# jyakaranda/A-LeGO-LOAM

Hardware: AMD Instinct MI355X
Metric: scans/sec (16x1800 LiDAR) full IP->LO->LM loop (higher is better)
Workload: dtype f32/f64

## Files before the change

### a-lego-loam_amd/csrc/kernels_lm.hip

```cpp
#include "dev_cost.h"
#include "prof.h"
#include "kf_store.h"
#include "gmap.h"
#include "vgrid.h"

#define LM_BLOCK 256

DEV_INLINE double* ldp(const LmCtx& L, int slot) { return L.ld + (size_t)slot * LD_COUNT; }
DEV_INLINE int* lip(const LmCtx& L, int slot) { return L.li + (size_t)slot * LI_COUNT; }

DEV_INLINE void lm_map_update(const LmCtx& L, int slot, int* li, int merge) {
  const int nkf = li[LI_NKF];
  if (nkf == 0) return;
  int* rec = L.rec + (size_t)slot * L.K;
  const int cnt = li[LI_REC_CNT];
  bool changed = false;
  if (cnt < L.K) {
    const int nk = min(nkf, L.K);
    changed = li[LI_DIRTY] != 0;
    for (int j = 0; j < nk; ++j) rec[j] = nkf - nk + j;
    li[LI_REC_CNT] = nk;
  } else if (li[LI_LATEST] != nkf - 1) {
    for (int j = 0; j + 1 < L.K; ++j) rec[j] = rec[j + 1];
    rec[L.K - 1] = nkf - 1;
// ... 82 lines not shown
  if (j >= nk) return;
  const int* rec = L.rec + (size_t)slot * L.K;
  int offc = 0, offs = 0;
  for (int i = 0; i < j; ++i) { const int* kc = kf_cnt_of(L, kf_row(L, slot, rec[i])); offc += kc[KF_CORNER]; offs += kc[KF_SURF] + kc[KF_OUTL]; }
  const KfRingRow R = kf_ring_row_at(L, slot, kf_entry(L, rec[j]), KF_CORNER);
  const int nc = R.cnt[KF_CORNER], ns = R.cnt[KF_SURF], no = R.cnt[KF_OUTL];
  float m[3][4];
  keypose_matrix(R.pose, m);
  const float4 *sc_ = R.raw, *ss_ = kf_raw_of(L, R.row, KF_SURF), *so_ = kf_raw_of(L, R.row, KF_OUTL);
  float4* dc = L.map_corner_raw + (size_t)slot * L.map_cap_c + offc;
  float4* ds = L.map_surf_raw + (size_t)slot * L.map_cap_s + offs;
  for (int i = blockIdx.x * LM_BLOCK + threadIdx.x; i < nc; i += gridDim.x * LM_BLOCK) dc[i] = kf_transform(m, sc_[i]);
  for (int i = blockIdx.x * LM_BLOCK + threadIdx.x; i < ns; i += gridDim.x * LM_BLOCK) ds[i] = kf_transform(m, ss_[i]);
  for (int i = blockIdx.x * LM_BLOCK + threadIdx.x; i < no; i += gridDim.x * LM_BLOCK) ds[ns + i] = kf_transform(m, so_[i]);
  if (j == nk - 1 && blockIdx.x == 0 && threadIdx.x == 0) { li[LI_KRAW_C] = offc + nc; li[LI_KRAW_S] = offs + ns + no; }
}

__global__ void __launch_bounds__(LM_BLOCK) lm_total(DevCtx d, LmCtx L) {
  const int slot = blockIdx.y + d.slot0;
  int* li = lip(L, slot);
  if (!li[LI_RUN]) return;
  int ns = li[LI_NCUR_S], no = li[LI_NCUR_O];
  if (ns + no > L.total_cap) { no = L.total_cap - ns; if (threadIdx.x == 0 && blockIdx.x == 0) li[LI_OVERFLOW] = 1; }
  const float4* s = L.cur_surf_ds + (size_t)slot * L.kf_cap_s;
  const float4* o = L.cur_outl_ds + (size_t)slot * L.kf_cap_o;
  float4* t = L.cur_total + (size_t)slot * L.total_cap;
  for (int i = blockIdx.x * LM_BLOCK + threadIdx.x; i < ns; i += gridDim.x * LM_BLOCK) t[i] = s[i];
  for (int i = blockIdx.x * LM_BLOCK + threadIdx.x; i < no; i += gridDim.x * LM_BLOCK) t[ns + i] = o[i];
  if (blockIdx.x == 0 && threadIdx.x == 0) li[LI_NTOTAL] = ns + no;
}

DEV_INLINE int cell_coord(float x, float inv) { return (int)fminf(fmaxf(floorf(x * inv), -1073741824.0f), 1073741824.0f); }
DEV_INLINE int grid_cell(const GridGeom& g, float x, float y, float z, int* cx, int* cy, int* cz) {
  int ix = cell_coord(x, g.inv) - g.ox, iy = cell_coord(y, g.inv) - g.oy, iz = cell_coord(z, g.inv) - g.oz;
  *cx = ix; *cy = iy; *cz = iz;
  ix = min(max(ix, 0), g.gx - 1); iy = min(max(iy, 0), g.gy - 1); iz = min(max(iz, 0), g.gz - 1);
  return ix + g.gx * (iy + g.gy * iz);
}

__global__ void __launch_bounds__(LM_BLOCK) lm_grid_build(DevCtx d, LmCtx L) {
  const int slot = blockIdx.y + d.slot0, m = blockIdx.x;
  const int* li = lip(L, slot);
  if (!li[LI_REBUILD]) return;
  __shared__ GridGeom s_g;
// ... 782 lines not shown
  return hipFuncSetAttribute(reinterpret_cast<const void*>(lm_solve), hipFuncAttributeMaxDynamicSharedMemorySize, (int)LM_SOLVE_DYN_BYTES) == hipSuccess ? 0 : -1;
}

void launch_lm_prepare(const DevCtx& d, const LmCtx& L, int stage, int run_hint, int par, hipStream_t st) {
  const bool small = run_hint == 0 || stage == 2;
  const dim3 grid = small ? dim3(1, 1, d.n_launch) : dim3(8, 3, d.n_launch);
  ALEGO_LAUNCH(lm_prepare, grid, dim3(small ? 64 : LM_BLOCK), 0, st, d, L, stage, run_hint, par);
}
void launch_lm_stage(const DevCtx& d, const LmCtx& L, int run_hint, int par, hipStream_t st) {
  const dim3 grid = run_hint == 0 ? dim3(1, 1, d.n_launch) : dim3(8, 3, d.n_launch);
  ALEGO_LAUNCH(lm_stage, grid, dim3(run_hint == 0 ? 64 : LM_BLOCK), 0, st, d, L, run_hint, par);
}
void launch_lm_concat(const DevCtx& d, const LmCtx& L, hipStream_t st) {
  ALEGO_LAUNCH(lm_concat, dim3(2, L.K, d.n_launch), dim3(LM_BLOCK), 0, st, d, L);
}
void launch_lm_total(const DevCtx& d, const LmCtx& L, hipStream_t st) {
  ALEGO_LAUNCH(lm_total, dim3(8, d.n_launch), dim3(LM_BLOCK), 0, st, d, L);
}
void launch_lm_grid(const DevCtx& d, const LmCtx& L, hipStream_t st) {
  ALEGO_LAUNCH(lm_grid_build, dim3(2, d.n_launch), dim3(LM_BLOCK), 0, st, d, L);
}
int launch_lm_register(const DevCtx& d, const LmCtx& L, hipStream_t st, int (*allreduce)(void*, double*, size_t, hipStream_t), void* ar_ctx) {
  ALEGO_LAUNCH(lm_knn, dim3(lm_reg_grid(d, LM_ASSOC_GX)), dim3(128), 0, st, d, L);
  ALEGO_LAUNCH(lm_fit, dim3(lm_reg_grid(d, LM_FIT_GX)), dim3(128), 0, st, d, L);
  if (allreduce) {
    double* part = L.shard_part + (size_t)d.slot0 * 32;
    const size_t cnt = (size_t)d.n_launch * 32;
    const dim3 g1((d.n_launch + 63) / 64), b1(64);
    const int pre_next = d.P.lm_max_iters <= 0 ? (int)LM_PRE_STEP_FIRST_NEXT : (int)LM_PRE_STEP_NEXT;
    for (int outer = 0; outer < d.P.lm_outer_iters; ++outer) {
      ALEGO_LAUNCH(lm_shard_eval, dim3(d.n_launch), dim3(LM_SOLVE_T), LM_SOLVE_RED_BYTES, st, d, L, 0, outer == 0 ? (int)LM_PRE_PACK : pre_next);
      if (int rc = allreduce(ar_ctx, part, cnt, st)) return rc;
      for (int it = 0; it < d.P.lm_max_iters; ++it) {
// ... 21 lines not shown
```

### a-lego-loam_amd/csrc/kernels_voxel.hip

```cpp
#include <algorithm>
#include <cstring>

#include <hip/hip_runtime.h>

#include <vector>

#include "voxel.h"
#include "wave.h"
#include "vgrid.h"
#include "guard_alloc.h"
#include "prof.h"

typedef unsigned long long u64;

__device__ __forceinline__ bool vx_enabled(const VoxJob& J) { return J.enable == nullptr || *J.enable != 0; }

#ifndef VX_SMALL_MAX
#define VX_SMALL_MAX 8192
#endif

#ifndef VG_T
#define VG_T 512
#endif
#define VG_W (VG_T / 64)
#define VG_DMAX 9
#define VG_ND (1 << VG_DMAX)
#define VG_U 4

__device__ __forceinline__ int vg_div(int pos, int seglen, double inv_seglen) {
  int q = (int)((double)pos * inv_seglen);
  if (q * seglen > pos) --q;
  if ((q + 1) * seglen <= pos) ++q;
  return q;
}

#ifdef ALEGO_TIMING
__device__ long long vg_times[16];
#define VG_TICK(k) do { if (threadIdx.x == 0 && blockIdx.x == 0) vg_times[k] = wall_clock64(); } while (0)
#else
#define VG_TICK(k)
#endif
#define VG_LDS_BYTES ((2 * VG_W * VG_ND + VG_ND + 6 * VG_W + VG_W + 2 * (VG_W + 1)) * 4)
__device__ void vox_big_job(const VoxCtx& V, int job, unsigned char* smem) {
  const VoxJob J = V.jobs[job];
  const int n = min(*J.n_in, J.cap);
  const int tid = threadIdx.x, lane = tid & 63, wave = tid >> 6;
  typedef int cnt_t[VG_W][VG_ND];
  cnt_t* s_cnt = reinterpret_cast<cnt_t*>(smem);
  int* s_tot = reinterpret_cast<int*>(smem) + 2 * VG_W * VG_ND;
  typedef float red_t[VG_W];
  red_t* s_red = reinterpret_cast<red_t*>(s_tot + VG_ND);
  int* s_w = reinterpret_cast<int*>(s_red + 6);
  int* s_wbase = s_w + VG_W;
  int* s_nextfirst = s_wbase + VG_W + 1;
  const float inv = 1.0f / J.leaf;
  VG_TICK(0);
  float mn[3] = {3.402823466e+38f, 3.402823466e+38f, 3.402823466e+38f}, mx[3] = {-3.402823466e+38f, -3.402823466e+38f, -3.402823466e+38f};
  for (int i0 = tid; i0 < n; i0 += VG_T * VG_U) {
    float4 p[VG_U];
#pragma unroll
    for (int k = 0; k < VG_U; ++k) p[k] = J.in[min(i0 + k * VG_T, n - 1)];
#pragma unroll
    for (int k = 0; k < VG_U; ++k) vgr_box_add(mn, mx, p[k]);
  }
#pragma unroll
  for (int a = 0; a < 3; ++a) {
    bfly_minmax_f32(mn[a], mx[a]);
    if (lane == 0) { s_red[a][wave] = mn[a]; s_red[3 + a][wave] = mx[a]; }
  }
  __syncthreads();
#pragma unroll
  for (int a = 0; a < 3; ++a) {
    mn[a] = s_red[a][0]; mx[a] = s_red[3 + a][0];
#pragma unroll
    for (int w = 1; w < VG_W; ++w) { mn[a] = fminf(mn[a], s_red[a][w]); mx[a] = fmaxf(mx[a], s_red[3 + a][w]); }
  }
  if (tid < 3) {
    unsigned* bb = V.bbox + job * 8;
    bb[tid] = vgr_enc(tid == 0 ? mn[0] : tid == 1 ? mn[1] : mn[2]);
    bb[4 + tid] = ~vgr_enc(tid == 0 ? mx[0] : tid == 1 ? mx[1] : mx[2]);
  }
  const int sel = (J.mode == 1 && J.out_sel) ? *J.out_sel : 0;
  float4* const outp = J.out + (size_t)sel * (J.mode == 1 ? J.out_stride : 0);
  if (J.mode == 1 && tid < 6 && J.box_out) J.box_out[(size_t)sel * 8 + (tid < 3 ? tid : tid + 1)] = tid == 0 ? mn[0] : tid == 1 ? mn[1] : tid == 2 ? mn[2] : tid == 3 ? mx[0] : tid == 4 ? mx[1] : mx[2];
  if (vgr_leaf_too_small(mn, mx, inv)) {
    for (int i = tid; i < min(n, J.out_cap); i += VG_T) outp[i] = J.in[i];
    if (tid == 0) { *J.n_out = min(n, J.out_cap); if (n > J.out_cap && J.overflow) *J.overflow = 1;
                    if (J.mode == 1 && J.n_sel_out) J.n_sel_out[(size_t)sel * J.n_sel_stride] = min(n, J.out_cap); }
    return;
  }
  const VgrGeom g = vgr_geom(mn, mx, inv);
  const int bits = max(vgr_bits(g.T), 1);
  const int P = (bits + VG_DMAX - 1) / VG_DMAX, D = (bits + P - 1) / P, nd = 1 << D;
  const unsigned dmask = (unsigned)(nd - 1);
  const int seglen = ((n + VG_T - 1) / VG_T) * 64;
  const double inv_seglen = 1.0 / (double)seglen;
  const int seg0 = min(n, wave * seglen), seg1 = min(n, seg0 + seglen);
  unsigned* keys = V.keys + J.off;
  u64* bufA = V.pairs_a + J.off;
  u64* bufB = V.pairs_b + J.off;
  VG_TICK(1);
  for (int q = lane; q < VG_ND; q += 64) { s_cnt[0][wave][q] = 0; }
  for (int r0 = seg0 + lane; r0 < seg1; r0 += 64 * VG_U) {
    float4 pt[VG_U];
#pragma unroll
    for (int k = 0; k < VG_U; ++k) pt[k] = J.in[min(r0 + 64 * k, n - 1)];
#pragma unroll
    for (int k = 0; k < VG_U; ++k) {
      const int i = r0 + 64 * k;
      if (i < seg1) {
        const unsigned key = vgr_id(g, pt[k], inv);
        keys[i] = key;
        atomicAdd(&s_cnt[0][wave][key & dmask], 1);
      }
    }
  }
  VG_TICK(2);
  for (int p = 0; p < P; ++p) {
    const int cur = p & 1, nxt = cur ^ 1;
    const int sh = p * D, shn = (p + 1) * D;
    const u64* src = (p & 1) ? bufA : bufB;
// ... 46 lines not shown
        if (valid) {
          const int pos = my[dg] + s_tot[dg] + rank;
          dst[pos] = e[k];
          if (p + 1 < P) atomicAdd(&s_cnt[nxt][vg_div(pos, seglen, inv_seglen)][(key >> shn) & dmask], 1);
        }
        if (valid && rank == 0) my[dg] += (int)__popcll(m);
      }
    }
    VG_TICK(4 + 2 * p);
  }
  const u64* srt = (P & 1) ? bufA : bufB;
  __threadfence_block();
  __syncthreads();
  VG_TICK(11);
  if (J.mode == 1) {
    for (int i = tid; i < min(n, J.out_cap); i += VG_T) outp[i] = J.in[(unsigned)srt[i]];
    if (tid == 0) { *J.n_out = min(n, J.out_cap); if (n > J.out_cap && J.overflow) *J.overflow = 1;
                    if (J.n_sel_out) J.n_sel_out[(size_t)sel * J.n_sel_stride] = min(n, J.out_cap); }
    __syncthreads();
    return;
  }
  auto head_rounds = [&](int r0, bool* head) {
    u64 cur[VG_U], prv[VG_U];
#pragma unroll
    for (int k = 0; k < VG_U; ++k) {
      const int i = r0 + 64 * k + lane;
      cur[k] = srt[min(i, n - 1)]; prv[k] = srt[max(min(i, n - 1) - 1, 0)];
    }
#pragma unroll
    for (int k = 0; k < VG_U; ++k) {
      const int i = r0 + 64 * k + lane;
// ... 28 lines not shown
  VG_TICK(12);
  for (int r = tid; r < min(nvox, J.out_cap); r += VG_T) {
    int w = 0;
#pragma unroll
    for (int q = 1; q < VG_W; ++q) w += (r >= s_wbase[q]) ? 1 : 0;
    const int loc = r - s_wbase[w], ws0 = min(n, w * seglen);
    const int a = hl[ws0 + loc], bn = hl[ws0 + min(loc + 1, s_w[w] - 1)];
    const int b = loc + 1 < s_w[w] ? bn : s_nextfirst[w + 1];
    float sx = 0.f, sy = 0.f, sz = 0.f, si = 0.f;
    for (int j = a; j < b; j += 8) {
      unsigned q[8];
      float4 pt[8];
#pragma unroll
      for (int k = 0; k < 8; ++k) q[k] = (unsigned)srt[min(j + k, b - 1)];
#pragma unroll
      for (int k = 0; k < 8; ++k) pt[k] = J.in[q[k]];
#pragma unroll
      for (int k = 0; k < 8; ++k) if (j + k < b) { sx += pt[k].x; sy += pt[k].y; sz += pt[k].z; si += pt[k].w; }
    }
    const float fn = (float)(b - a);
    J.out[r] = make_float4(sx / fn, sy / fn, sz / fn, si / fn);
  }
  if (tid == 0) { *J.n_out = min(nvox, J.out_cap); if (nvox > J.out_cap && J.overflow) *J.overflow = 1; }
  __syncthreads();
  VG_TICK(13);
}
#ifdef ALEGO_TIMING
extern "C" void alego_vg_times(long long* out) { (void)hipMemcpyFromSymbol(out, HIP_SYMBOL(vg_times), sizeof(long long) * 16); }
#endif

#define VX_SB 512
#define VS_W (VX_SB / 64)
#define VS_DMAX 9
#define VS_ND (1 << VS_DMAX)
__device__ __forceinline__ bool vx_less(const unsigned* key, unsigned a, unsigned b) { return key[a] < key[b] || (key[a] == key[b] && a < b); }

__device__ void vox_small_job(const VoxCtx& V, int job) {
  const VoxJob J = V.jobs[job];
  const int n = min(*J.n_in, J.cap);
  const int tid = threadIdx.x, lane = tid & 63, wave = tid >> 6;
  extern __shared__ __attribute__((aligned(16))) unsigned char vs_smem[];
  unsigned* s_key = reinterpret_cast<unsigned*>(vs_smem);
  unsigned short* s_ia = reinterpret_cast<unsigned short*>(vs_smem + 4 * VX_SMALL_MAX);
  unsigned short* s_ib = reinterpret_cast<unsigned short*>(vs_smem + 6 * VX_SMALL_MAX);
  unsigned short* s_cnt = reinterpret_cast<unsigned short*>(vs_smem + 8 * VX_SMALL_MAX);
  __shared__ float s_red[6][VX_SB / 64];
  __shared__ int s_scan[VX_SB / 64];
  __shared__ int s_tot[VS_ND];
  const int sel = (J.mode == 1 && J.out_sel) ? *J.out_sel : 0;
  float4* const outp = J.out + (size_t)sel * (J.mode == 1 ? J.out_stride : 0);
  if (n == 0) { if (tid == 0) { *J.n_out = 0; if (J.mode == 1 && J.n_sel_out) J.n_sel_out[(size_t)sel * J.n_sel_stride] = 0; } return; }
  const float inv = 1.0f / J.leaf;
  VG_TICK(0);
  float mn[3] = {3.402823466e+38f, 3.402823466e+38f, 3.402823466e+38f}, mx[3] = {-3.402823466e+38f, -3.402823466e+38f, -3.402823466e+38f};
  for (int i = tid; i < n; i += VX_SB) vgr_box_add(mn, mx, J.in[i]);
#pragma unroll
  for (int a = 0; a < 3; ++a) {
    bfly_minmax_f32(mn[a], mx[a]);
    if (lane == 0) { s_red[a][wave] = mn[a]; s_red[3 + a][wave] = mx[a]; }
  }
  __syncthreads();
#pragma unroll
  for (int a = 0; a < 3; ++a) {
    mn[a] = s_red[a][0]; mx[a] = s_red[3 + a][0];
#pragma unroll
    for (int w = 1; w < VX_SB / 64; ++w) { mn[a] = fminf(mn[a], s_red[a][w]); mx[a] = fmaxf(mx[a], s_red[3 + a][w]); }
  }
  if (tid < 3) {
    unsigned* bb = V.bbox + job * 8;
    bb[tid] = vgr_enc(tid == 0 ? mn[0] : tid == 1 ? mn[1] : mn[2]);
    bb[4 + tid] = ~vgr_enc(tid == 0 ? mx[0] : tid == 1 ? mx[1] : mx[2]);
  }
  if (J.mode == 1 && tid < 6 && J.box_out) J.box_out[(size_t)sel * 8 + (tid < 3 ? tid : tid + 1)] = tid == 0 ? mn[0] : tid == 1 ? mn[1] : tid == 2 ? mn[2] : tid == 3 ? mx[0] : tid == 4 ? mx[1] : mx[2];
  if (vgr_leaf_too_small(mn, mx, inv)) {
    for (int i = tid; i < min(n, J.out_cap); i += VX_SB) outp[i] = J.in[i];
    if (tid == 0) { *J.n_out = min(n, J.out_cap); if (n > J.out_cap && J.overflow) *J.overflow = 1;
                    if (J.mode == 1 && J.n_sel_out) J.n_sel_out[(size_t)sel * J.n_sel_stride] = min(n, J.out_cap); }
    return;
  }
  VG_TICK(1);
  const VgrGeom g = vgr_geom(mn, mx, inv);
  for (int i = tid; i < n; i += VX_SB) s_key[i] = vgr_id(g, J.in[i], inv);
  VG_TICK(2);
  const int bits = max(vgr_bits(g.T), 1);
  const int P = (bits + VS_DMAX - 1) / VS_DMAX, D = (bits + P - 1) / P, nd = 1 << D;
  const unsigned dmask = (unsigned)(nd - 1);
  const int seglen = ((n + VX_SB - 1) / VX_SB) * 64;
  const int seg0 = min(n, wave * seglen), seg1 = min(n, seg0 + seglen);
  unsigned short* my = s_cnt + wave * VS_ND;
  for (int p = 0; p < P; ++p) {
    const unsigned short* src = (p & 1) ? s_ia : s_ib;
    unsigned short* dst = (p & 1) ? s_ib : s_ia;
    const int sh = p * D;
    __syncthreads();
    for (int q = lane; q < nd; q += 64) my[q] = 0;
    for (int sweep = 0; sweep < 2; ++sweep) {
      if (sweep == 1) {
        __syncthreads();
        if (tid < nd) {
          int run = 0;
#pragma unroll
          for (int w = 0; w < VS_W; ++w) { const int c = s_cnt[w * VS_ND + tid]; s_cnt[w * VS_ND + tid] = (unsigned short)run; run += c; }
          s_tot[tid] = run;
        }
        __syncthreads();
        if (wave == 0) {
          constexpr int PER = VS_ND / 64;
          int v[PER], sum = 0;
#pragma unroll
          for (int k = 0; k < PER; ++k) { const int dgt = lane * PER + k; v[k] = dgt < nd ? s_tot[dgt] : 0; sum += v[k]; }
          const int incl = wave_incl_scan(sum);
          int run = incl - sum;
#pragma unroll
          for (int k = 0; k < PER; ++k) { const int dgt = lane * PER + k; if (dgt < nd) s_tot[dgt] = run; run += v[k]; }
        }
        __syncthreads();
      }
      for (int r0 = seg0; r0 < seg1; r0 += 64) {
        const int i = r0 + lane;
        const bool valid = i < seg1;
        const unsigned idx = valid ? (p == 0 ? (unsigned)i : (unsigned)src[i]) : 0u;
        const unsigned dg = valid ? (s_key[idx] >> sh) & dmask : 0u;
        unsigned long long m = __ballot(valid);
        for (int bit = 0; bit < D; ++bit) {
          const bool one = (dg >> bit) & 1u;
          const unsigned long long bal = __ballot(one);
          m &= one ? bal : ~bal;
        }
        const int rank = (int)__builtin_amdgcn_mbcnt_hi((unsigned)(m >> 32), __builtin_amdgcn_mbcnt_lo((unsigned)m, 0u));
        if (sweep == 1 && valid) dst[(int)my[dg] + s_tot[dg] + rank] = (unsigned short)idx;
        if (valid && rank == 0) my[dg] = (unsigned short)(my[dg] + (int)__popcll(m));
      }
    }
  }
  __syncthreads();
  const unsigned short* srt = (P & 1) ? s_ia : s_ib;
  unsigned short* hl = (P & 1) ? s_ib : s_ia;
  VG_TICK(3);
  if (J.mode == 1) {
    for (int i = tid; i < min(n, J.out_cap); i += VX_SB) outp[i] = J.in[srt[i]];
    if (tid == 0) { *J.n_out = min(n, J.out_cap); if (n > J.out_cap && J.overflow) *J.overflow = 1;
                    if (J.n_sel_out) J.n_sel_out[(size_t)sel * J.n_sel_stride] = min(n, J.out_cap); }
    __syncthreads();
    return;
  }
  int heads = 0;
  for (int r0 = seg0; r0 < seg1; r0 += 64) {
    const int i = r0 + lane;
    const bool head = i < seg1 && (i == 0 || s_key[srt[i]] != s_key[srt[i - 1]]);
    heads += (int)__popcll(__ballot(head));
  }
  if (lane == 0) s_scan[wave] = heads;
  __syncthreads();
  int vbase = 0, nvox = 0;
#pragma unroll
// ... 3 lines not shown
    const bool head = i < seg1 && (i == 0 || s_key[srt[i]] != s_key[srt[i - 1]]);
    const unsigned long long hb = __ballot(head);
    if (head) hl[vbase + (int)__builtin_amdgcn_mbcnt_hi((unsigned)(hb >> 32), __builtin_amdgcn_mbcnt_lo((unsigned)hb, 0u))] = (unsigned short)i;
    vbase += (int)__popcll(hb);
  }
  __syncthreads();
  VG_TICK(4);
  VG_TICK(5);
  VG_TICK(6);
  for (int r = tid; r < min(nvox, J.out_cap); r += VX_SB) {
    const int a = hl[r], b = r + 1 < nvox ? (int)hl[r + 1] : n;
    float sx = 0.f, sy = 0.f, sz = 0.f, si = 0.f;
    for (int j = a; j < b; j += 4) {
      float4 pt[4];
#pragma unroll
      for (int k = 0; k < 4; ++k) pt[k] = J.in[srt[min(j + k, b - 1)]];
#pragma unroll
      for (int k = 0; k < 4; ++k) if (j + k < b) { sx += pt[k].x; sy += pt[k].y; sz += pt[k].z; si += pt[k].w; }
    }
    const float fn = (float)(b - a);
    J.out[r] = make_float4(sx / fn, sy / fn, sz / fn, si / fn);
  }
  if (tid == 0) { *J.n_out = min(nvox, J.out_cap); if (nvox > J.out_cap && J.overflow) *J.overflow = 1; }
  __syncthreads();
  VG_TICK(7);
}
__global__ void __launch_bounds__(VX_SB) vox_small(VoxCtx V) {
  extern __shared__ __attribute__((aligned(16))) unsigned char vs_smem_k[];
  const int cnt = V.cnt[0];
  for (int j = blockIdx.x; j < cnt; j += gridDim.x) {
    vox_small_job(V, V.list_small[j]);
    __syncthreads();
  }
  const int nbig = V.cnt[1];
  if ((int)blockIdx.x < V.grid_big) {
    for (int j = blockIdx.x; j < nbig; j += min((int)gridDim.x, V.grid_big)) {
      vox_big_job(V, V.list_big[j], vs_smem_k);
      __syncthreads();
    }
  }
}

__global__ void __launch_bounds__(256) vox_plan(VoxCtx V) {
  __shared__ int s_n[2];
  if (threadIdx.x < 2) s_n[threadIdx.x] = 0;
  __syncthreads();
  for (int j = threadIdx.x; j < V.njobs; j += 256) {
    const VoxJob J = V.jobs[j];
    if (!vx_enabled(J)) continue;
    const int n = min(*J.n_in, J.cap);
    if (n == 0) { *J.n_out = 0; if (J.mode == 1 && J.n_sel_out) J.n_sel_out[(size_t)(J.out_sel ? *J.out_sel : 0) * J.n_sel_stride] = 0; continue; }
    if (n <= VX_SMALL_MAX) V.list_small[atomicAdd(&s_n[0], 1)] = j;
    else V.list_big[atomicAdd(&s_n[1], 1)] = j;
  }
  __syncthreads();
  if (threadIdx.x < 2) V.cnt[threadIdx.x] = s_n[threadIdx.x];
}

#define VX_SMALL_LDS (8 * VX_SMALL_MAX + 2 * VS_W * VS_ND)
int vox_create(VoxCtx* V, const VoxJob* jobs, int njobs, std::string* err) {
  std::memset(V, 0, sizeof(*V));
  if (hipFuncSetAttribute(reinterpret_cast<const void*>(vox_small), hipFuncAttributeMaxDynamicSharedMemorySize, VX_SMALL_LDS) != hipSuccess) { *err = "vox_create: hipFuncSetAttribute"; return -2; }
  std::vector<VoxJob> h(jobs, jobs + njobs);
  size_t total = 0;
  for (auto& j : h) {
    j.off = (int)total;
// ... 31 lines not shown
```

### a-lego-loam_amd/csrc/lm_ctx.h

```cpp
#ifndef ALEGO_LM_CTX_H_
#define ALEGO_LM_CTX_H_
#include "dev_common.h"

enum {
  LI_NKF = 0,
  LI_DIRTY,
  LI_RUN,
  LI_REBUILD,
  LI_FRAME,
  LI_FLAGS,
  LI_NCC, LI_NSC,
  LI_SUM0, LI_SUM1,
  LI_KF_ADDED, LI_OPTIMIZED,
  LI_KRAW_C, LI_KRAW_S, LI_KDS_C, LI_KDS_S,
  LI_NIN_C, LI_NIN_S, LI_NIN_O,
  LI_NCUR_C, LI_NCUR_S, LI_NCUR_O,
  LI_NTOTAL, LI_NTOTAL_DS,
  LI_NREBUILD,
  LI_OVERFLOW,
  LI_REC_CNT,
  LI_LATEST,
  LI_NU_C, LI_NU_S,
  LI_UVALID,
  LI_PREV_CNT,
// ... 82 lines not shown
  unsigned long long *U_c, *U_s;
  int *Ucnt_c, *Ucnt_s;
  int* rec_prev;
  float4* newkeys;
  int shard_rank, shard_world;
  double* shard_part;
  void* shard_state;
  int* shard_ctl;
  unsigned* map_bbox;
  float4 *kf_raw_c, *kf_raw_s, *kf_raw_o;
  int* rec;
  int* kf_cnt;
  float* kf_pose;
  float4 *map_corner_raw, *map_surf_raw;
  float4 *map_corner_ds, *map_surf_ds;
  float4 *cur_corner_ds, *cur_surf_ds, *cur_outl_ds, *cur_total, *cur_total_ds;
  GridGeom* grid;
  int *cell_start, *cell_cur;
  float4* cell_pts;
  const unsigned* vox_bbox;
  int vox_slot0;
  int* knn;
  double* blocks;
  double* crows;
  int arc_frames_cap, arc_points_cap;
  float4* arc_pts;
  int* arc_tab;
  float* arc_pose;
  int* arc_stat;
  double* arc_stamp;
  int* arc_stamped;
// ... 11 lines not shown
```

### a-lego-loam_amd/csrc/lm_host.hip

```cpp
#include "lm_host.h"
#include "guard_alloc.h"

#include <cstdio>
#include <cstdlib>
#include <algorithm>
#include <cstring>
#include <vector>

#include <rccl/rccl.h>

#include "kf_store.h"
#include "voxel.h"
#include "gmap.h"
#include "loc_math.h"

void launch_lm_prepare(const DevCtx& d, const LmCtx& L, int stage, int run_hint, int par, hipStream_t st);
void launch_lm_stage(const DevCtx& d, const LmCtx& L, int run_hint, int par, hipStream_t st);
void launch_lm_concat(const DevCtx& d, const LmCtx& L, hipStream_t st);
void launch_lm_total(const DevCtx& d, const LmCtx& L, hipStream_t st);
void launch_lm_grid(const DevCtx& d, const LmCtx& L, hipStream_t st);
int launch_lm_register(const DevCtx& d, const LmCtx& L, hipStream_t st, int (*allreduce)(void*, double*, size_t, hipStream_t), void* ar_ctx);
size_t lm_solve_row_bytes_max();
size_t lm_solve_row_bytes_default();
void launch_lm_retransform(const DevCtx& d, const LmCtx& L, int ring, hipStream_t st);
void launch_map_update(const DevCtx& d, const LmCtx& L, const MapWork& W, hipStream_t st);
void launch_map_accum(const DevCtx& d, const LmCtx& L, const MapWork& W, hipStream_t st);
void launch_lm_apply_correction(const DevCtx& d, const LmCtx& L, int slot, const double* rc_dev, hipStream_t st);
void launch_pg_apply(const LmCtx& L, const int* apply_dev, int n_slots, hipStream_t st);
void launch_pg_retransform(const LmCtx& L, const int* apply_dev, int slot0, int n, int j, hipStream_t st);
void launch_pg_sorted(const LmCtx& L, const int* apply_dev, int slot0, int n, int all, hipStream_t st);
void launch_loc_select(const DevCtx& d, const LmCtx& L, hipStream_t st);

struct LmHost {
  alego_params P;
  int n_slots;
  int gsize;
  std::vector<hipStream_t> st;
  LmCtx L;
  std::vector<VoxCtx> vm, v2;
  std::vector<VoxCtx> vk;
  std::vector<MapWork> work;
  bool fallback_ok = true;
  ncclComm_t comm = nullptr;
  std::string dist_err;
  std::vector<void*> allocs;
  std::vector<long> frames;
  GvCtx gv;
  int* arc_off = nullptr;
  VoxCtx vloc;
  bool vloc_made = false;
};

namespace {
template <class T>
bool A(LmHost* lm, T** p, size_t count, std::string* err) {
  void* q = nullptr;
  size_t bytes = count * sizeof(T);
// ... 71 lines not shown
  ok = ok && A(lm, &L.stage_odom, B * 2 * 8, err);
  ok = ok && A(lm, &L.in_corner, B * L.in_cap_c, err) && A(lm, &L.in_surf, B * L.in_cap_s, err) && A(lm, &L.in_outl, B * L.in_cap_o, err);
  ok = ok && ring_alloc(lm, L, B * L.KR, err);
  ok = ok && A(lm, &L.kf_tmp_c, B * L.kf_cap_c, err) && A(lm, &L.kf_tmp_s, B * L.total_cap, err);
  ok = ok && A(lm, &L.rec, B * L.K, err) && A(lm, &L.rec_prev, B * L.K, err);
  ok = ok && A(lm, &L.U_c, B * L.map_cap_c, err) && A(lm, &L.U_s, B * L.map_cap_s, err) && A(lm, &L.Ucnt_c, B * L.map_cap_c, err) && A(lm, &L.Ucnt_s, B * L.map_cap_s, err);
  ok = ok && A(lm, &L.newkeys, B * 2 * L.total_cap, err) && A(lm, &L.map_bbox, B * 2 * 8, err);
  {
    double* part = nullptr; int* ctl = nullptr; double* state = nullptr;
    ok = ok && A(lm, &part, B * 32, err) && A(lm, &ctl, B * 8, err) && A(lm, &state, B * 64, err);
    L.shard_part = part; L.shard_ctl = ctl; L.shard_state = state;
  }
  ok = ok && A(lm, &L.map_corner_raw, lm->fallback_ok ? B * L.map_cap_c : 1, err) && A(lm, &L.map_surf_raw, lm->fallback_ok ? B * L.map_cap_s : 1, err);
  ok = ok && A(lm, &L.map_corner_ds, B * L.map_cap_c, err) && A(lm, &L.map_surf_ds, B * L.map_cap_s, err);
  ok = ok && A(lm, &L.cur_corner_ds, B * L.kf_cap_c, err) && A(lm, &L.cur_surf_ds, B * L.kf_cap_s, err) && A(lm, &L.cur_outl_ds, B * L.kf_cap_o, err);
  ok = ok && A(lm, &L.cur_total, B * L.total_cap, err) && A(lm, &L.cur_total_ds, B * L.total_cap, err);
  ok = ok && A(lm, &L.grid, B * 2, err) && A(lm, &L.cell_start, B * 2 * ((size_t)L.gcap + 1), err) && A(lm, &L.cell_cur, B * 2 * ((size_t)L.gcap + 1), err);
  ok = ok && A(lm, &L.cell_pts, B * 2 * L.map_cap_s, err);
  ok = ok && A(lm, &L.blocks, B * L.qcap * 8, err) && A(lm, &L.crows, B * L.qcap * 10, err) && A(lm, &L.knn, B * L.qcap * 5, err);
  if (!ok) { lm_host_destroy(lm); return nullptr; }
  std::vector<double> ld(B * LD_COUNT, 0.0);
  for (size_t b = 0; b < B; ++b) { ld[b * LD_COUNT + LD_Q_M2O] = 1.0; ld[b * LD_COUNT + LD_Q_O2L] = 1.0; ld[b * LD_COUNT + LD_Q_M2L] = 1.0; }
  if (hipMemcpy(L.ld, ld.data(), ld.size() * sizeof(double), hipMemcpyHostToDevice) != hipSuccess) { *err = "lm_host_create: upload failed"; lm_host_destroy(lm); return nullptr; }
  std::vector<int> li0(B * LI_COUNT, 0);
  for (size_t b = 0; b < B; ++b) li0[b * LI_COUNT + LI_LATEST] = -1;
  if (hipMemcpy(L.li, li0.data(), li0.size() * sizeof(int), hipMemcpyHostToDevice) != hipSuccess) { *err = "lm_host_create: upload failed"; lm_host_destroy(lm); return nullptr; }
  for (size_t g = 0; g < st.size(); ++g) {
  std::vector<VoxJob> jm, j1, j2, jk;
  for (size_t b = g * gsize; b < B && b < (g + 1) * (size_t)gsize; ++b) {
    int* li = L.li + b * LI_COUNT;
    if (lm->fallback_ok) {
      jm.push_back(VoxJob{L.map_corner_raw + b * L.map_cap_c, li + LI_KRAW_C, L.map_corner_ds + b * L.map_cap_c, li + LI_KDS_C, li + LI_REBUILD_FB, P.lm_leaf_corner, L.map_cap_c, L.map_cap_c, li + LI_OVERFLOW, 0});
      jm.push_back(VoxJob{L.map_surf_raw + b * L.map_cap_s, li + LI_KRAW_S, L.map_surf_ds + b * L.map_cap_s, li + LI_KDS_S, li + LI_REBUILD_FB, P.lm_leaf_surf, L.map_cap_s, L.map_cap_s, li + LI_OVERFLOW, 0});
    }
    j1.push_back(VoxJob{L.in_corner + b * L.in_cap_c, li + LI_NIN_C, L.cur_corner_ds + b * L.kf_cap_c, li + LI_NCUR_C, li + LI_RUN, P.lm_leaf_corner, L.in_cap_c, L.kf_cap_c, li + LI_OVERFLOW, 0});
    j1.push_back(VoxJob{L.in_surf + b * L.in_cap_s, li + LI_NIN_S, L.cur_surf_ds + b * L.kf_cap_s, li + LI_NCUR_S, li + LI_RUN, P.lm_leaf_surf, L.in_cap_s, L.kf_cap_s, li + LI_OVERFLOW, 0});
    j1.push_back(VoxJob{L.in_outl + b * L.in_cap_o, li + LI_NIN_O, L.cur_outl_ds + b * L.kf_cap_o, li + LI_NCUR_O, li + LI_RUN, P.lm_leaf_outlier, L.in_cap_o, L.kf_cap_o, li + LI_OVERFLOW, 0});
    j2.push_back(VoxJob{L.cur_total + b * L.total_cap, li + LI_NTOTAL, L.cur_total_ds + b * L.total_cap, li + LI_NTOTAL_DS, li + LI_RUN, P.lm_leaf_surf, L.total_cap, L.total_cap, li + LI_OVERFLOW, 0});
    kf_sort_jobs(L, P, (int)b, &jk);
  }
  const int ns = (int)j1.size() / 3;
  jm.insert(jm.end(), j1.begin(), j1.end());
  jm.insert(jm.end(), jk.begin(), jk.end());
  if (vox_create(&lm->vm[g], jm.data(), (int)jm.size(), err) || vox_create(&lm->v2[g], j2.data(), (int)j2.size(), err) ||
      vox_create(&lm->vk[g], jk.data(), (int)jk.size(), err)) { lm_host_destroy(lm); return nullptr; }
  const bool big_scans = d.N > 8 * 8192;
  lm->vm[g].grid_small = 3 * ns + std::max(2, ns / 2);
  if (const char* e = getenv("ALEGO_VOX_GRID_DIV")) { const int dv = std::max(1, atoi(e)); lm->vm[g].grid_small = std::max(2, lm->vm[g].grid_small / dv); lm->v2[g].grid_small = std::max(1, lm->v2[g].grid_small / dv); }
  lm->vm[g].grid_big = (!d.opt_map_merge || big_scans) ? std::max(2, ns / 2) : std::min(8, std::max(2, ns / 2));
  lm->v2[g].grid_big = big_scans ? std::max(2, ns / 2) : std::max(1, ns / 16);
  lm->vk[g].grid_small = 2; lm->vk[g].grid_big = 2;
  MapWork& W = lm->work[g];
  W.cap = std::max(4096, 64 * ns);
  if (!A(lm, &W.items, (size_t)W.cap, err) || !A(lm, &W.count, 2, err)) { lm_host_destroy(lm); return nullptr; }
  }
  return lm;
}

void lm_host_destroy(LmHost* lm) {
  if (!lm) return;
  if (lm->comm) { (void)ncclCommDestroy(lm->comm); lm->comm = nullptr; }
  for (auto& v : lm->vm) vox_destroy(&v);
// ... 60 lines not shown
    par = (int)(A->k & 1);
    if (A->k >= 2 && hipStreamWaitEvent(A->front, A->back_same, 0) != hipSuccess) { *err = "hipStreamWaitEvent failed"; return ALEGO_ERR_HIP; }
    if (hint != 0 && A->k >= 1 && hipStreamWaitEvent(A->front, A->back_other, 0) != hipSuccess) { *err = "hipStreamWaitEvent failed"; return ALEGO_ERR_HIP; }
    launch_lm_stage(d, L, hint, par, A->front);
    if (hipEventRecord(A->staged, A->front) != hipSuccess || hipStreamWaitEvent(st, A->staged, 0) != hipSuccess) { *err = "event hand-over to the LaserMapping stream failed"; return ALEGO_ERR_HIP; }
    stage = 2;
  }
  launch_lm_prepare(d, L, stage, hint, par, st);
  if (!dbg_sync(st, "lm_prepare", err)) return ALEGO_ERR_HIP;
  if (n_run == 0) return 0;
  if (L.loc_on) {
    launch_loc_select(d, L, st);
    if (!dbg_sync(st, "loc_select", err)) return ALEGO_ERR_HIP;
  }
  if (int r = map_sequence(lm, d, L, g, st, err)) return r;
  launch_lm_total(d, L, st);
  if (int r = vox_run(lm->v2[g], st, err)) return r;
  if (!dbg_sync(st, "vox total", err)) return ALEGO_ERR_HIP;
  if (int r = launch_lm_register(d, L, st, lm->comm ? &lm_allreduce : nullptr, lm)) { *err = "sharded registration: " + lm->dist_err; return r; }
  if (!dbg_sync(st, "lm_register", err)) return ALEGO_ERR_HIP;
  return 0;
}

static void clear_run_flags_outside(LmHost* lm, const DevCtx& d) {
  const int g = d.slot0 / lm->gsize;
  const int lo = g * lm->gsize, hi = std::min(lm->n_slots, lo + lm->gsize);
  if (d.slot0 == lo && d.slot0 + d.n_launch == hi) return;
  for (int s = lo; s < hi; ++s) {
    if (s >= d.slot0 && s < d.slot0 + d.n_launch) continue;
    (void)hipMemsetAsync(lm->L.li + (size_t)s * LI_COUNT + LI_RUN, 0, sizeof(int), lm->st[g]);
  }
}

// ... 572 lines not shown
```

### a-lego-loam_amd/csrc/voxel.h

```cpp
#ifndef ALEGO_VOXEL_H_
#define ALEGO_VOXEL_H_
#include <hip/hip_runtime.h>

#include <string>

struct VoxJob {
  const float4* in;
  const int* n_in;
  float4* out;
  int* n_out;
  const int* enable;
  float leaf;
  int cap;
  int out_cap;
  int* overflow;
  int off;
  int mode;
  const int* out_sel;
  int out_stride;
  float* box_out;
  int* n_sel_out;
  int n_sel_stride;
};

struct VoxCtx {
  VoxJob* jobs;
  int njobs;
  unsigned* bbox;
  unsigned* keys;
  unsigned long long *pairs_a, *pairs_b;
  int *list_small, *list_big, *cnt;
  int grid_small, grid_big;
  unsigned total;
};

int vox_create(VoxCtx* V, const VoxJob* jobs, int njobs, std::string* err);
void vox_destroy(VoxCtx* V);
// ... 4 lines not shown
```

Baseline: 444,200.

## Chain total-cloud voxel job into first voxel pass and read surf+outlier inputs directly

Removes the lm_total concatenation kernel and its buffer. The total-cloud voxel filter now reads the surface and outlier downsampled clouds directly through a two-input VoxJob. For small scans the surf, outlier and total jobs are chained inside one block of the first voxel launch, which drops a separate vox_run and a kernel launch. The small-job radix sort also keeps per-point digit, rank and peer data in registers instead of re-running the ballot sweep, and launch bounds now request occupancy. The cost is extra branching on every point load and serialized chained stages within a block.

Result: no change. 445,600 (median of 5 runs) (+0.3%).

```diff
diff --git a/a-lego-loam_amd/csrc/kernels_lm.hip b/a-lego-loam_amd/csrc/kernels_lm.hip
--- a/a-lego-loam_amd/csrc/kernels_lm.hip
+++ b/a-lego-loam_amd/csrc/kernels_lm.hip
@@ -120,20 +120,6 @@
   for (int i = blockIdx.x * LM_BLOCK + threadIdx.x; i < ns; i += gridDim.x * LM_BLOCK) ds[i] = kf_transform(m, ss_[i]);
   for (int i = blockIdx.x * LM_BLOCK + threadIdx.x; i < no; i += gridDim.x * LM_BLOCK) ds[ns + i] = kf_transform(m, so_[i]);
   if (j == nk - 1 && blockIdx.x == 0 && threadIdx.x == 0) { li[LI_KRAW_C] = offc + nc; li[LI_KRAW_S] = offs + ns + no; }
-}
-
-__global__ void __launch_bounds__(LM_BLOCK) lm_total(DevCtx d, LmCtx L) {
-  const int slot = blockIdx.y + d.slot0;
-  int* li = lip(L, slot);
-  if (!li[LI_RUN]) return;
-  int ns = li[LI_NCUR_S], no = li[LI_NCUR_O];
-  if (ns + no > L.total_cap) { no = L.total_cap - ns; if (threadIdx.x == 0 && blockIdx.x == 0) li[LI_OVERFLOW] = 1; }
-  const float4* s = L.cur_surf_ds + (size_t)slot * L.kf_cap_s;
-  const float4* o = L.cur_outl_ds + (size_t)slot * L.kf_cap_o;
-  float4* t = L.cur_total + (size_t)slot * L.total_cap;
-  for (int i = blockIdx.x * LM_BLOCK + threadIdx.x; i < ns; i += gridDim.x * LM_BLOCK) t[i] = s[i];
-  for (int i = blockIdx.x * LM_BLOCK + threadIdx.x; i < no; i += gridDim.x * LM_BLOCK) t[ns + i] = o[i];
-  if (blockIdx.x == 0 && threadIdx.x == 0) li[LI_NTOTAL] = ns + no;
 }
 
 DEV_INLINE int cell_coord(float x, float inv) { return (int)fminf(fmaxf(floorf(x * inv), -1073741824.0f), 1073741824.0f); }
@@ -946,9 +932,6 @@
 void launch_lm_concat(const DevCtx& d, const LmCtx& L, hipStream_t st) {
   ALEGO_LAUNCH(lm_concat, dim3(2, L.K, d.n_launch), dim3(LM_BLOCK), 0, st, d, L);
 }
-void launch_lm_total(const DevCtx& d, const LmCtx& L, hipStream_t st) {
-  ALEGO_LAUNCH(lm_total, dim3(8, d.n_launch), dim3(LM_BLOCK), 0, st, d, L);
-}
 void launch_lm_grid(const DevCtx& d, const LmCtx& L, hipStream_t st) {
   ALEGO_LAUNCH(lm_grid_build, dim3(2, d.n_launch), dim3(LM_BLOCK), 0, st, d, L);
 }
diff --git a/a-lego-loam_amd/csrc/kernels_voxel.hip b/a-lego-loam_amd/csrc/kernels_voxel.hip
--- a/a-lego-loam_amd/csrc/kernels_voxel.hip
+++ b/a-lego-loam_amd/csrc/kernels_voxel.hip
@@ -14,6 +14,18 @@
 typedef unsigned long long u64;
 
 __device__ __forceinline__ bool vx_enabled(const VoxJob& J) { return J.enable == nullptr || *J.enable != 0; }
+__device__ __forceinline__ int vx_count(const VoxJob& J, int* n0, bool* over) {
+  *n0 = min(*J.n_in, J.cap); *over = false;
+  if (J.in2 == nullptr) return *n0;
+  int n1 = min(*J.n_in2, J.cap2);
+  if (*n0 + n1 > J.cap) { n1 = J.cap - *n0; *over = true; }
+  return *n0 + n1;
+}
+__device__ __forceinline__ float4 vx_in(const VoxJob& J, int n0, int i) { return i < n0 ? J.in[i] : J.in2[i - n0]; }
+__device__ __forceinline__ void vx_note_input(const VoxJob& J, int n, bool over) {
+  if (J.n_cat) *J.n_cat = n;
+  if (over && J.overflow) *J.overflow = 1;
+}
 
 #ifndef VX_SMALL_MAX
 #define VX_SMALL_MAX 8192
@@ -43,8 +55,10 @@
 #define VG_LDS_BYTES ((2 * VG_W * VG_ND + VG_ND + 6 * VG_W + VG_W + 2 * (VG_W + 1)) * 4)
 __device__ void vox_big_job(const VoxCtx& V, int job, unsigned char* smem) {
   const VoxJob J = V.jobs[job];
-  const int n = min(*J.n_in, J.cap);
+  int n0; bool over;
+  const int n = vx_count(J, &n0, &over);
   const int tid = threadIdx.x, lane = tid & 63, wave = tid >> 6;
+  if (tid == 0) vx_note_input(J, n, over);
   typedef int cnt_t[VG_W][VG_ND];
   cnt_t* s_cnt = reinterpret_cast<cnt_t*>(smem);
   int* s_tot = reinterpret_cast<int*>(smem) + 2 * VG_W * VG_ND;
@@ -59,7 +73,7 @@
   for (int i0 = tid; i0 < n; i0 += VG_T * VG_U) {
     float4 p[VG_U];
 #pragma unroll
-    for (int k = 0; k < VG_U; ++k) p[k] = J.in[min(i0 + k * VG_T, n - 1)];
+    for (int k = 0; k < VG_U; ++k) p[k] = vx_in(J, n0, min(i0 + k * VG_T, n - 1));
 #pragma unroll
     for (int k = 0; k < VG_U; ++k) vgr_box_add(mn, mx, p[k]);
   }
@@ -84,7 +98,7 @@
   float4* const outp = J.out + (size_t)sel * (J.mode == 1 ? J.out_stride : 0);
   if (J.mode == 1 && tid < 6 && J.box_out) J.box_out[(size_t)sel * 8 + (tid < 3 ? tid : tid + 1)] = tid == 0 ? mn[0] : tid == 1 ? mn[1] : tid == 2 ? mn[2] : tid == 3 ? mx[0] : tid == 4 ? mx[1] : mx[2];
   if (vgr_leaf_too_small(mn, mx, inv)) {
-    for (int i = tid; i < min(n, J.out_cap); i += VG_T) outp[i] = J.in[i];
+    for (int i = tid; i < min(n, J.out_cap); i += VG_T) outp[i] = vx_in(J, n0, i);
     if (tid == 0) { *J.n_out = min(n, J.out_cap); if (n > J.out_cap && J.overflow) *J.overflow = 1;
                     if (J.mode == 1 && J.n_sel_out) J.n_sel_out[(size_t)sel * J.n_sel_stride] = min(n, J.out_cap); }
     return;
@@ -104,7 +118,7 @@
   for (int r0 = seg0 + lane; r0 < seg1; r0 += 64 * VG_U) {
     float4 pt[VG_U];
 #pragma unroll
-    for (int k = 0; k < VG_U; ++k) pt[k] = J.in[min(r0 + 64 * k, n - 1)];
+    for (int k = 0; k < VG_U; ++k) pt[k] = vx_in(J, n0, min(r0 + 64 * k, n - 1));
 #pragma unroll
     for (int k = 0; k < VG_U; ++k) {
       const int i = r0 + 64 * k;
@@ -181,7 +195,7 @@
   __syncthreads();
   VG_TICK(11);
   if (J.mode == 1) {
-    for (int i = tid; i < min(n, J.out_cap); i += VG_T) outp[i] = J.in[(unsigned)srt[i]];
+    for (int i = tid; i < min(n, J.out_cap); i += VG_T) outp[i] = vx_in(J, n0, (int)(unsigned)srt[i]);
     if (tid == 0) { *J.n_out = min(n, J.out_cap); if (n > J.out_cap && J.overflow) *J.overflow = 1;
                     if (J.n_sel_out) J.n_sel_out[(size_t)sel * J.n_sel_stride] = min(n, J.out_cap); }
     __syncthreads();
@@ -240,7 +254,7 @@
 #pragma unroll
       for (int k = 0; k < 8; ++k) q[k] = (unsigned)srt[min(j + k, b - 1)];
 #pragma unroll
-      for (int k = 0; k < 8; ++k) pt[k] = J.in[q[k]];
+      for (int k = 0; k < 8; ++k) pt[k] = vx_in(J, n0, (int)q[k]);
 #pragma unroll
       for (int k = 0; k < 8; ++k) if (j + k < b) { sx += pt[k].x; sy += pt[k].y; sz += pt[k].z; si += pt[k].w; }
     }
@@ -257,14 +271,19 @@
 
 #define VX_SB 512
 #define VS_W (VX_SB / 64)
+#define VS_R (VX_SMALL_MAX / VX_SB)
+#define VX_WAVES_PER_SIMD 4
+static_assert(VX_SMALL_MAX % VX_SB == 0 && VX_SMALL_MAX <= 65536, "vox_small_job: whole rounds per wavefront, 16-bit point order");
 #define VS_DMAX 9
 #define VS_ND (1 << VS_DMAX)
 __device__ __forceinline__ bool vx_less(const unsigned* key, unsigned a, unsigned b) { return key[a] < key[b] || (key[a] == key[b] && a < b); }
 
 __device__ void vox_small_job(const VoxCtx& V, int job) {
   const VoxJob J = V.jobs[job];
-  const int n = min(*J.n_in, J.cap);
+  int n0; bool over;
+  const int n = vx_count(J, &n0, &over);
   const int tid = threadIdx.x, lane = tid & 63, wave = tid >> 6;
+  if (tid == 0) vx_note_input(J, n, over);
   extern __shared__ __attribute__((aligned(16))) unsigned char vs_smem[];
   unsigned* s_key = reinterpret_cast<unsigned*>(vs_smem);
   unsigned short* s_ia = reinterpret_cast<unsigned short*>(vs_smem + 4 * VX_SMALL_MAX);
@@ -279,7 +298,7 @@
   const float inv = 1.0f / J.leaf;
   VG_TICK(0);
   float mn[3] = {3.402823466e+38f, 3.402823466e+38f, 3.402823466e+38f}, mx[3] = {-3.402823466e+38f, -3.402823466e+38f, -3.402823466e+38f};
-  for (int i = tid; i < n; i += VX_SB) vgr_box_add(mn, mx, J.in[i]);
+  for (int i = tid; i < n; i += VX_SB) vgr_box_add(mn, mx, vx_in(J, n0, i));
 #pragma unroll
   for (int a = 0; a < 3; ++a) {
     bfly_minmax_f32(mn[a], mx[a]);
@@ -299,14 +318,14 @@
   }
   if (J.mode == 1 && tid < 6 && J.box_out) J.box_out[(size_t)sel * 8 + (tid < 3 ? tid : tid + 1)] = tid == 0 ? mn[0] : tid == 1 ? mn[1] : tid == 2 ? mn[2] : tid == 3 ? mx[0] : tid == 4 ? mx[1] : mx[2];
   if (vgr_leaf_too_small(mn, mx, inv)) {
-    for (int i = tid; i < min(n, J.out_cap); i += VX_SB) outp[i] = J.in[i];
+    for (int i = tid; i < min(n, J.out_cap); i += VX_SB) outp[i] = vx_in(J, n0, i);
     if (tid == 0) { *J.n_out = min(n, J.out_cap); if (n > J.out_cap && J.overflow) *J.overflow = 1;
                     if (J.mode == 1 && J.n_sel_out) J.n_sel_out[(size_t)sel * J.n_sel_stride] = min(n, J.out_cap); }
     return;
   }
   VG_TICK(1);
   const VgrGeom g = vgr_geom(mn, mx, inv);
-  for (int i = tid; i < n; i += VX_SB) s_key[i] = vgr_id(g, J.in[i], inv);
+  for (int i = tid; i < n; i += VX_SB) s_key[i] = vgr_id(g, vx_in(J, n0, i), inv);
   VG_TICK(2);
   const int bits = max(vgr_bits(g.T), 1);
   const int P = (bits + VS_DMAX - 1) / VS_DMAX, D = (bits + P - 1) / P, nd = 1 << D;
@@ -320,29 +339,11 @@
     const int sh = p * D;
     __syncthreads();
     for (int q = lane; q < nd; q += 64) my[q] = 0;
-    for (int sweep = 0; sweep < 2; ++sweep) {
-      if (sweep == 1) {
-        __syncthreads();
-        if (tid < nd) {
-          int run = 0;
-#pragma unroll
-          for (int w = 0; w < VS_W; ++w) { const int c = s_cnt[w * VS_ND + tid]; s_cnt[w * VS_ND + tid] = (unsigned short)run; run += c; }
-          s_tot[tid] = run;
-        }
-        __syncthreads();
-        if (wave == 0) {
-          constexpr int PER = VS_ND / 64;
-          int v[PER], sum = 0;
-#pragma unroll
-          for (int k = 0; k < PER; ++k) { const int dgt = lane * PER + k; v[k] = dgt < nd ? s_tot[dgt] : 0; sum += v[k]; }
-          const int incl = wave_incl_scan(sum);
-          int run = incl - sum;
-#pragma unroll
-          for (int k = 0; k < PER; ++k) { const int dgt = lane * PER + k; if (dgt < nd) s_tot[dgt] = run; run += v[k]; }
-        }
-        __syncthreads();
-      }
-      for (int r0 = seg0; r0 < seg1; r0 += 64) {
+    unsigned pk[VS_R];
+#pragma unroll
+    for (int r = 0; r < VS_R; ++r) {
+      const int r0 = seg0 + 64 * r;
+      if (r0 < seg1) {
         const int i = r0 + lane;
         const bool valid = i < seg1;
         const unsigned idx = valid ? (p == 0 ? (unsigned)i : (unsigned)src[i]) : 0u;
@@ -353,9 +354,40 @@
           const unsigned long long bal = __ballot(one);
           m &= one ? bal : ~bal;
         }
-        const int rank = (int)__builtin_amdgcn_mbcnt_hi((unsigned)(m >> 32), __builtin_amdgcn_mbcnt_lo((unsigned)m, 0u));
-        if (sweep == 1 && valid) dst[(int)my[dg] + s_tot[dg] + rank] = (unsigned short)idx;
-        if (valid && rank == 0) my[dg] = (unsigned short)(my[dg] + (int)__popcll(m));
+        const unsigned rank = __builtin_amdgcn_mbcnt_hi((unsigned)(m >> 32), __builtin_amdgcn_mbcnt_lo((unsigned)m, 0u));
+        const unsigned peers = (unsigned)__popcll(m);
+        pk[r] = dg | (rank << VS_DMAX) | (peers << (VS_DMAX + 6));
+        if (valid && rank == 0) my[dg] = (unsigned short)(my[dg] + peers);
+      }
+    }
+    __syncthreads();
+    if (tid < nd) {
+      int run = 0;
+#pragma unroll
+      for (int w = 0; w < VS_W; ++w) { const int c = s_cnt[w * VS_ND + tid]; s_cnt[w * VS_ND + tid] = (unsigned short)run; run += c; }
+      s_tot[tid] = run;
+    }
+    __syncthreads();
+    if (wave == 0) {
+      constexpr int PER = VS_ND / 64;
+      int v[PER], sum = 0;
+#pragma unroll
+      for (int k = 0; k < PER; ++k) { const int dgt = lane * PER + k; v[k] = dgt < nd ? s_tot[dgt] : 0; sum += v[k]; }
+      const int incl = wave_incl_scan(sum);
+      int run = incl - sum;
+#pragma unroll
+      for (int k = 0; k < PER; ++k) { const int dgt = lane * PER + k; if (dgt < nd) s_tot[dgt] = run; run += v[k]; }
+    }
+    __syncthreads();
+#pragma unroll
+    for (int r = 0; r < VS_R; ++r) {
+      const int r0 = seg0 + 64 * r;
+      if (r0 < seg1) {
+        const int i = r0 + lane;
+        const bool valid = i < seg1;
+        const unsigned dg = pk[r] & (VS_ND - 1), rank = (pk[r] >> VS_DMAX) & 63u, peers = pk[r] >> (VS_DMAX + 6);
+        if (valid) dst[(int)my[dg] + s_tot[dg] + (int)rank] = p == 0 ? (unsigned short)i : src[i];
+        if (valid && rank == 0) my[dg] = (unsigned short)(my[dg] + peers);
       }
     }
   }
@@ -364,7 +396,7 @@
   unsigned short* hl = (P & 1) ? s_ib : s_ia;
   VG_TICK(3);
   if (J.mode == 1) {
-    for (int i = tid; i < min(n, J.out_cap); i += VX_SB) outp[i] = J.in[srt[i]];
+    for (int i = tid; i < min(n, J.out_cap); i += VX_SB) outp[i] = vx_in(J, n0, (int)srt[i]);
     if (tid == 0) { *J.n_out = min(n, J.out_cap); if (n > J.out_cap && J.overflow) *J.overflow = 1;
                     if (J.n_sel_out) J.n_sel_out[(size_t)sel * J.n_sel_stride] = min(n, J.out_cap); }
     __syncthreads();
@@ -398,7 +430,7 @@
     for (int j = a; j < b; j += 4) {
       float4 pt[4];
 #pragma unroll
-      for (int k = 0; k < 4; ++k) pt[k] = J.in[srt[min(j + k, b - 1)]];
+      for (int k = 0; k < 4; ++k) pt[k] = vx_in(J, n0, (int)srt[min(j + k, b - 1)]);
 #pragma unroll
       for (int k = 0; k < 4; ++k) if (j + k < b) { sx += pt[k].x; sy += pt[k].y; sz += pt[k].z; si += pt[k].w; }
     }
@@ -409,18 +441,23 @@
   __syncthreads();
   VG_TICK(7);
 }
-__global__ void __launch_bounds__(VX_SB) vox_small(VoxCtx V) {
+__global__ void __launch_bounds__(VX_SB, VX_WAVES_PER_SIMD) vox_small(VoxCtx V) {
   extern __shared__ __attribute__((aligned(16))) unsigned char vs_smem_k[];
-  const int cnt = V.cnt[0];
-  for (int j = blockIdx.x; j < cnt; j += gridDim.x) {
-    vox_small_job(V, V.list_small[j]);
-    __syncthreads();
-  }
-  const int nbig = V.cnt[1];
-  if ((int)blockIdx.x < V.grid_big) {
-    for (int j = blockIdx.x; j < nbig; j += min((int)gridDim.x, V.grid_big)) {
-      vox_big_job(V, V.list_big[j], vs_smem_k);
-      __syncthreads();
+#pragma unroll 1
+  for (int big = 0; big < 2; ++big) {
+    const int cnt = V.cnt[big];
+    const int* list = big ? V.list_big : V.list_small;
+    const int groups = big ? min((int)gridDim.x, V.grid_big) : (int)gridDim.x;
+    if ((int)blockIdx.x >= groups) break;
+    for (int k = blockIdx.x; k < cnt; k += groups) {
+      const int head = list[k], stages = max(V.jobs[head].chain, 1);
+      for (int job = head; job < head + stages; ++job) {
+        const VoxJob& J = V.jobs[job];
+        int n0; bool over;
+        if (vx_count(J, &n0, &over) <= VX_SMALL_MAX) vox_small_job(V, job);
+        else vox_big_job(V, job, vs_smem_k);
+        __syncthreads();
+      }
     }
   }
 }
@@ -431,9 +468,11 @@
   __syncthreads();
   for (int j = threadIdx.x; j < V.njobs; j += 256) {
     const VoxJob J = V.jobs[j];
-    if (!vx_enabled(J)) continue;
-    const int n = min(*J.n_in, J.cap);
-    if (n == 0) { *J.n_out = 0; if (J.mode == 1 && J.n_sel_out) J.n_sel_out[(size_t)(J.out_sel ? *J.out_sel : 0) * J.n_sel_stride] = 0; continue; }
+    if (J.chain < 0 || !vx_enabled(J)) continue;
+    if (J.chain > 0) { V.list_small[atomicAdd(&s_n[0], 1)] = j; continue; }
+    int n0; bool over;
+    const int n = vx_count(J, &n0, &over);
+    if (n == 0) { *J.n_out = 0; vx_note_input(J, 0, false); if (J.mode == 1 && J.n_sel_out) J.n_sel_out[(size_t)(J.out_sel ? *J.out_sel : 0) * J.n_sel_stride] = 0; continue; }
     if (n <= VX_SMALL_MAX) V.list_small[atomicAdd(&s_n[0], 1)] = j;
     else V.list_big[atomicAdd(&s_n[1], 1)] = j;
   }
diff --git a/a-lego-loam_amd/csrc/lm_ctx.h b/a-lego-loam_amd/csrc/lm_ctx.h
--- a/a-lego-loam_amd/csrc/lm_ctx.h
+++ b/a-lego-loam_amd/csrc/lm_ctx.h
@@ -120,7 +120,7 @@
   float* kf_pose;
   float4 *map_corner_raw, *map_surf_raw;
   float4 *map_corner_ds, *map_surf_ds;
-  float4 *cur_corner_ds, *cur_surf_ds, *cur_outl_ds, *cur_total, *cur_total_ds;
+  float4 *cur_corner_ds, *cur_surf_ds, *cur_outl_ds, *cur_total_ds;
   GridGeom* grid;
   int *cell_start, *cell_cur;
   float4* cell_pts;
diff --git a/a-lego-loam_amd/csrc/lm_host.hip b/a-lego-loam_amd/csrc/lm_host.hip
--- a/a-lego-loam_amd/csrc/lm_host.hip
+++ b/a-lego-loam_amd/csrc/lm_host.hip
@@ -17,7 +17,6 @@
 void launch_lm_prepare(const DevCtx& d, const LmCtx& L, int stage, int run_hint, int par, hipStream_t st);
 void launch_lm_stage(const DevCtx& d, const LmCtx& L, int run_hint, int par, hipStream_t st);
 void launch_lm_concat(const DevCtx& d, const LmCtx& L, hipStream_t st);
-void launch_lm_total(const DevCtx& d, const LmCtx& L, hipStream_t st);
 void launch_lm_grid(const DevCtx& d, const LmCtx& L, hipStream_t st);
 int launch_lm_register(const DevCtx& d, const LmCtx& L, hipStream_t st, int (*allreduce)(void*, double*, size_t, hipStream_t), void* ar_ctx);
 size_t lm_solve_row_bytes_max();
@@ -41,6 +40,7 @@
   std::vector<VoxCtx> vk;
   std::vector<MapWork> work;
   bool fallback_ok = true;
+  bool chained = true;
   ncclComm_t comm = nullptr;
   std::string dist_err;
   std::vector<void*> allocs;
@@ -142,7 +142,7 @@
   ok = ok && A(lm, &L.map_corner_raw, lm->fallback_ok ? B * L.map_cap_c : 1, err) && A(lm, &L.map_surf_raw, lm->fallback_ok ? B * L.map_cap_s : 1, err);
   ok = ok && A(lm, &L.map_corner_ds, B * L.map_cap_c, err) && A(lm, &L.map_surf_ds, B * L.map_cap_s, err);
   ok = ok && A(lm, &L.cur_corner_ds, B * L.kf_cap_c, err) && A(lm, &L.cur_surf_ds, B * L.kf_cap_s, err) && A(lm, &L.cur_outl_ds, B * L.kf_cap_o, err);
-  ok = ok && A(lm, &L.cur_total, B * L.total_cap, err) && A(lm, &L.cur_total_ds, B * L.total_cap, err);
+  ok = ok && A(lm, &L.cur_total_ds, B * L.total_cap, err);
   ok = ok && A(lm, &L.grid, B * 2, err) && A(lm, &L.cell_start, B * 2 * ((size_t)L.gcap + 1), err) && A(lm, &L.cell_cur, B * 2 * ((size_t)L.gcap + 1), err);
   ok = ok && A(lm, &L.cell_pts, B * 2 * L.map_cap_s, err);
   ok = ok && A(lm, &L.blocks, B * L.qcap * 8, err) && A(lm, &L.crows, B * L.qcap * 10, err) && A(lm, &L.knn, B * L.qcap * 5, err);
@@ -153,6 +153,8 @@
   std::vector<int> li0(B * LI_COUNT, 0);
   for (size_t b = 0; b < B; ++b) li0[b * LI_COUNT + LI_LATEST] = -1;
   if (hipMemcpy(L.li, li0.data(), li0.size() * sizeof(int), hipMemcpyHostToDevice) != hipSuccess) { *err = "lm_host_create: upload failed"; lm_host_destroy(lm); return nullptr; }
+  const bool big_scans = d.N > 8 * 8192;
+  lm->chained = !big_scans;
   for (size_t g = 0; g < st.size(); ++g) {
   std::vector<VoxJob> jm, j1, j2, jk;
   for (size_t b = g * gsize; b < B && b < (g + 1) * (size_t)gsize; ++b) {
@@ -164,16 +166,22 @@
     j1.push_back(VoxJob{L.in_corner + b * L.in_cap_c, li + LI_NIN_C, L.cur_corner_ds + b * L.kf_cap_c, li + LI_NCUR_C, li + LI_RUN, P.lm_leaf_corner, L.in_cap_c, L.kf_cap_c, li + LI_OVERFLOW, 0});
     j1.push_back(VoxJob{L.in_surf + b * L.in_cap_s, li + LI_NIN_S, L.cur_surf_ds + b * L.kf_cap_s, li + LI_NCUR_S, li + LI_RUN, P.lm_leaf_surf, L.in_cap_s, L.kf_cap_s, li + LI_OVERFLOW, 0});
     j1.push_back(VoxJob{L.in_outl + b * L.in_cap_o, li + LI_NIN_O, L.cur_outl_ds + b * L.kf_cap_o, li + LI_NCUR_O, li + LI_RUN, P.lm_leaf_outlier, L.in_cap_o, L.kf_cap_o, li + LI_OVERFLOW, 0});
-    j2.push_back(VoxJob{L.cur_total + b * L.total_cap, li + LI_NTOTAL, L.cur_total_ds + b * L.total_cap, li + LI_NTOTAL_DS, li + LI_RUN, P.lm_leaf_surf, L.total_cap, L.total_cap, li + LI_OVERFLOW, 0});
+    VoxJob jt{L.cur_surf_ds + b * L.kf_cap_s, li + LI_NCUR_S, L.cur_total_ds + b * L.total_cap, li + LI_NTOTAL_DS, li + LI_RUN, P.lm_leaf_surf, L.total_cap, L.total_cap, li + LI_OVERFLOW, 0};
+    jt.in2 = L.cur_outl_ds + b * L.kf_cap_o; jt.n_in2 = li + LI_NCUR_O; jt.cap2 = L.kf_cap_o; jt.n_cat = li + LI_NTOTAL;
+    if (lm->chained) {
+      j1[j1.size() - 2].chain = 3; j1[j1.size() - 1].chain = -1; jt.chain = -1;
+      j1.push_back(jt);
+    } else {
+      j2.push_back(jt);
+    }
     kf_sort_jobs(L, P, (int)b, &jk);
   }
-  const int ns = (int)j1.size() / 3;
+  const int ns = (int)(B < (g + 1) * (size_t)gsize ? B - g * gsize : (size_t)gsize);
   jm.insert(jm.end(), j1.begin(), j1.end());
   jm.insert(jm.end(), jk.begin(), jk.end());
-  if (vox_create(&lm->vm[g], jm.data(), (int)jm.size(), err) || vox_create(&lm->v2[g], j2.data(), (int)j2.size(), err) ||
+  if (vox_create(&lm->vm[g], jm.data(), (int)jm.size(), err) || (!j2.empty() && vox_create(&lm->v2[g], j2.data(), (int)j2.size(), err)) ||
       vox_create(&lm->vk[g], jk.data(), (int)jk.size(), err)) { lm_host_destroy(lm); return nullptr; }
-  const bool big_scans = d.N > 8 * 8192;
-  lm->vm[g].grid_small = 3 * ns + std::max(2, ns / 2);
+  lm->vm[g].grid_small = (lm->chained ? 2 : 3) * ns + std::max(2, ns / 2);
   if (const char* e = getenv("ALEGO_VOX_GRID_DIV")) { const int dv = std::max(1, atoi(e)); lm->vm[g].grid_small = std::max(2, lm->vm[g].grid_small / dv); lm->v2[g].grid_small = std::max(1, lm->v2[g].grid_small / dv); }
   lm->vm[g].grid_big = (!d.opt_map_merge || big_scans) ? std::max(2, ns / 2) : std::min(8, std::max(2, ns / 2));
   lm->v2[g].grid_big = big_scans ? std::max(2, ns / 2) : std::max(1, ns / 16);
@@ -264,9 +272,10 @@
     if (!dbg_sync(st, "loc_select", err)) return ALEGO_ERR_HIP;
   }
   if (int r = map_sequence(lm, d, L, g, st, err)) return r;
-  launch_lm_total(d, L, st);
-  if (int r = vox_run(lm->v2[g], st, err)) return r;
-  if (!dbg_sync(st, "vox total", err)) return ALEGO_ERR_HIP;
+  if (!lm->chained) {
+    if (int r = vox_run(lm->v2[g], st, err)) return r;
+    if (!dbg_sync(st, "vox total", err)) return ALEGO_ERR_HIP;
+  }
   if (int r = launch_lm_register(d, L, st, lm->comm ? &lm_allreduce : nullptr, lm)) { *err = "sharded registration: " + lm->dist_err; return r; }
   if (!dbg_sync(st, "lm_register", err)) return ALEGO_ERR_HIP;
   return 0;
diff --git a/a-lego-loam_amd/csrc/voxel.h b/a-lego-loam_amd/csrc/voxel.h
--- a/a-lego-loam_amd/csrc/voxel.h
+++ b/a-lego-loam_amd/csrc/voxel.h
@@ -21,6 +21,11 @@
   float* box_out;
   int* n_sel_out;
   int n_sel_stride;
+  const float4* in2;
+  const int* n_in2;
+  int cap2;
+  int* n_cat;
+  int chain;
 };
 
 struct VoxCtx {
```
